# LSDOlab/femo_alpha

Measured on AMD Instinct MI355X. Metric: DOF/s (assembly+solve), forward solve of the RM shell; adjoint-gradient wallclock in adjoint_ms, higher is better.
Workload: dtype f64

## Files before the change

### femo_alpha_amd/_build.py

```python
from __future__ import annotations

import contextlib
import fcntl
import glob
import hashlib
import os
import shutil
import subprocess

CSRC = os.path.join(os.path.dirname(os.path.abspath(__file__)), "csrc")
INCLUDE = os.path.normpath(os.path.join(CSRC, "..", "..", "include"))
LIB = os.path.join(CSRC, "libfemo_hip.so")
HASHFILE = os.path.join(CSRC, "libfemo_hip.srchash")
SOURCES = ["femo_hip.hip"]
FLAGS = ["--offload-arch=gfx950", "-O3", "-std=c++17", "-fPIC", "-shared", "-munsafe-fp-atomics",
         "-Wno-unused-value"]


def dependencies():
    deps = sorted(glob.glob(os.path.join(CSRC, "*.hip")) + glob.glob(os.path.join(CSRC, "*.h"))
                  + [os.path.join(INCLUDE, "femo_hip.h")])
    return deps


# ... 51 lines not shown
            if os.path.exists(tmp):
                os.remove(tmp)
            raise RuntimeError("hipcc failed building libfemo_hip.so:\n" + res.stderr[-4000:])
        os.replace(tmp, LIB)
        _write_atomic(HASHFILE, digest + "\n")
    return LIB


SYM_LIB = os.path.join(CSRC, "libfemo_symbolic.so")
SYM_HASHFILE = os.path.join(CSRC, "libfemo_symbolic.srchash")
SYM_FLAGS = ["-O3", "-std=c++17", "-fPIC", "-shared", "-fopenmp"]


def symbolic_digest() -> str:
    h = hashlib.sha256(" ".join(SYM_FLAGS).encode())
    for d in (os.path.join(CSRC, "symbolic.cpp"), os.path.join(INCLUDE, "femo_symbolic.h")):
        h.update(os.path.basename(d).encode())
        with open(d, "rb") as fh:
            h.update(fh.read())
    return h.hexdigest()


def symbolic_needs_build() -> bool:
    if not os.path.exists(SYM_LIB) or not os.path.exists(SYM_HASHFILE):
        return True
    with open(SYM_HASHFILE) as fh:
        return fh.read().strip() != symbolic_digest()


def build_symbolic(force: bool = False) -> str:
    if not force and not symbolic_needs_build():
# ... 23 lines not shown
```

### femo_alpha_amd/csrc/femo_hip.hip

```cpp
#include "../../include/femo_hip.h"
#include "shell_device.h"
#include "frontal.h"
#include "sweeps_multi.h"
#include "shape_sens.h"
#include "residual_jvp.h"
#include "stress.h"
#include "stress_grad.h"
#include "stress_history.h"
#include "disp_history.h"
#include "ply_failure.h"
#include "ply_shear.h"
#include "field_jvp.h"
#include "ply_field_rev.h"
#include "layup.h"
#include "layup_mass.h"
#include "disp_aggregate.h"
#include "csr_map.h"
#include "hip_handles.h"

#include <hip/hip_runtime.h>

#include <algorithm>
#include <cmath>
#include <cstdio>
#include <cstdlib>
#include <cstring>
#include <string>
#include <utility>
#include <vector>

using namespace femo;

constexpr int WIDE_NP_DEFAULT = 512;
// ... 146 lines not shown
    DevBuf<double> scal;
    PinnedBuf<double> scal_host;
    bool jacobi_dirty = true;
    struct Options {
        int trailing = 0;
        int left_min = 64, left_max = 2048;
        int lookahead = 1, lookahead_cnt = 16;
        int super_panel = 512, super_panel_cnt = 64;
        int rows_fine_wg = 96;
        int narrow_fine_wg = 128;
        int fuse_rows = 1, fuse_rows_cnt = 2048;
        int fuse_rows_np = 2 * NBO;
        int sweep_graph = 0;
        int diag_v1_cnt = 512;
        int fused_schur = 1;
        int equilibrate = 0;
        int precond_nquad = 0;
        int grid_chunk = 32768;
        int wide_np = WIDE_NP_DEFAULT, wide_cnt = WIDE_CNT_DEFAULT;
        int strict = 1;
        int allow_pivot_repair = 0;
        int profile_verbose = 0;
        int diag_v1 = 0;
        int swork_slots = 8192;
        int xinv_small_cnt = 32;
        int bnd_tiled_nb = 1 << 30;
        int sweep_butterfly = 3;
        int sweep_w = 0;
        int assemble_fc = 1;
        int sweep_ahead = 2;
// ... 12 lines not shown
    double timing[5] = {0, 0, 0, 0, 0};
    std::string err;
    struct Frontal {
        bool ready = false, factored = false;
        bool have_factor = false;
        DevBuf<double> snap[6];
        bool snap_valid = false;
        bool w_mode = false;
        double* ahead_vec = nullptr;
        int ahead_levels = 0;
        bool x_inflight = false;
        int ntree = 0, nlevels = 0;
        std::vector<int> h_nf, h_npiv, h_level_off, h_level_nodes, h_level_maxnp, h_level_maxnb;
        std::vector<char> h_level_wide;
        DevBuf<int> nf, npiv, dofs, upmap, parent, left, right, level_nodes, elem_front, elem_map, info, cinv0, cinv1;
        DevBuf<long long> poff, soff, doff, linvoff, xoff;
        DevBuf<double> P, S, Linv, X, Xtmp, Swork;
        DevBuf<int> fel_off, fel;
        bool fc_ok = false;
        GraphExec sweep_graph;
        long long sweep_graph_key = -1;
        std::vector<long long> h_soff;
        long long p_doubles = 0, s_doubles = 0, linv_doubles = 0, x_doubles = 0;
        int swork_slots = 1;
        int max_nf = 0;
        int multi_nr = 4;
        double t_factor_ms = 0, t_assemble_ms = 0;
        int pivots_fixed = 0;
        bool profile = false;
        double prof_ms[8] = {0, 0, 0, 0, 0, 0, 0, 0};
// ... 449 lines not shown
    HIPCHK(c, hipStreamSynchronize(c->stream));
    float t_setup = 0, t_loop = 0;
    hipEventElapsedTime(&t_setup, c->ev[0], c->ev[1]);
    hipEventElapsedTime(&t_loop, c->ev[1], c->ev[2]);
    c->timing[0] = t_setup; c->timing[1] = t_loop; c->timing[2] = t_setup + t_loop; c->timing[3] = 0; c->timing[4] = napply;
    return finish_solve(c, "Jacobi-PCG", k, rr, bb, c->rtol * c->rtol * bb, iters, relres);
}


static FrontDev front_dev(const femo_ctx* c) {
    FrontDev fd;
    fd.ntree = c->fr.ntree; fd.nf = c->fr.nf; fd.npiv = c->fr.npiv; fd.poff = c->fr.poff; fd.soff = c->fr.soff; fd.doff = c->fr.doff;
    fd.dofs = c->fr.dofs; fd.upmap = c->fr.upmap; fd.parent = c->fr.parent; fd.child[0] = c->fr.left; fd.child[1] = c->fr.right;
    fd.linvoff = c->fr.linvoff; fd.xoff = c->fr.xoff; fd.P = c->fr.P; fd.S = c->fr.S; fd.Linv = c->fr.Linv; fd.X = c->fr.X; fd.Xtmp = c->fr.Xtmp;
    fd.cinv[0] = c->fr.cinv0; fd.cinv[1] = c->fr.cinv1;
    return fd;
}

struct ProfScope {
    femo_ctx* c; int cls; hipStream_t s; Event a, b;
    ProfScope(femo_ctx* c_, int cls_, hipStream_t s_ = nullptr) : c(c_), cls(cls_), s(s_ ? s_ : c_->stream.get()) {
        if (!c->fr.profile) return;
        hipEventCreate(a.out()); hipEventCreate(b.out());
        hipEventRecord(a, s);
    }
    ~ProfScope() {
        if (!c->fr.profile) return;
        hipEventRecord(b, s);
        c->fr.prof.push_back({std::move(a), std::move(b), cls, c->fr.cur_level, cls == 2 ? c->fr.last_fl : 0.0, cls == 2 ? c->fr.last_by : 0.0});
        c->fr.last_fl = c->fr.last_by = 0;
// ... 2017 lines not shown
    if (k == "trailing") { if (v < 0 || v > 2) return fail(c, "trailing: 0 auto, 1 left-looking, 2 right-looking"); o.trailing = v; }
    else if (k == "left_min") o.left_min = v;
    else if (k == "left_max") o.left_max = v;
    else if (k == "lookahead") o.lookahead = v != 0;
    else if (k == "lookahead_cnt") o.lookahead_cnt = v;
    else if (k == "super_panel") { if (v < 0) return fail(c, "super_panel: a column count (rounded down to whole 128-column panels; < 256 switches it off)"); o.super_panel = v; }
    else if (k == "super_panel_cnt") o.super_panel_cnt = v;
    else if (k == "rows_fine_wg") o.rows_fine_wg = v;
    else if (k == "narrow_fine_wg") o.narrow_fine_wg = v;
    else if (k == "diag_v1_cnt") o.diag_v1_cnt = v;
    else if (k == "sweep_graph") o.sweep_graph = v != 0;
    else if (k == "fuse_rows") o.fuse_rows = v != 0;
    else if (k == "fuse_rows_cnt") o.fuse_rows_cnt = v;
    else if (k == "fuse_rows_np") o.fuse_rows_np = v;
    else if (k == "fused_schur") o.fused_schur = v != 0;
    else if (k == "precond_nquad") { if (v != 0 && (v < 2 || v > 6)) return fail(c, "precond_nquad: 0 (the operator's rule) or 2..6"); o.precond_nquad = v; operator_changed(c); }
    else if (k == "equilibrate") { if (v < 0 || v > 2) return fail(c, "equilibrate: 0 off, 1 diag^-1/2, 2 nearest powers of two"); o.equilibrate = v; operator_changed(c); }
    else if (k == "grid_chunk") { if (v < 1 || v > 65535) return fail(c, "grid_chunk must be in 1..65535"); o.grid_chunk = v; }
    else if (k == "wide_np" || k == "wide_cnt") {
        if (c->fr.ready) return fail(c, "wide_np / wide_cnt shape the plan: set them before femo_set_frontal_plan");
        if (v < 0) return fail(c, "negative threshold");
        (k == "wide_np" ? o.wide_np : o.wide_cnt) = v;
    }
    else if (k == "strict") o.strict = v != 0;
    else if (k == "allow_pivot_repair") o.allow_pivot_repair = v != 0;
    else if (k == "stress_regularization") { if (value < 0) return fail(c, "stress_regularization: a coefficient >= 0 (the reference's is 0.5e3)"); c->stress_reg = value; }
    else if (k == "profile_verbose") o.profile_verbose = v != 0;
    else if (k == "diag_v1") { if (v < 0 || v > 3) return fail(c, "diag_v1: 0 auto, 1 round-2 kernel, 2 overlapped kernel, 3 the rule before the LDS diet"); o.diag_v1 = v; }
    else if (k == "profile") c->fr.profile = v != 0;
    else if (k == "bnd_tiled_nb") o.bnd_tiled_nb = v;
// ... 1133 lines not shown
    }
    {
        std::vector<int> inv0((size_t)ndofs_total, -1), inv1((size_t)ndofs_total, -1);
        for (int t = 0; t < ntree; ++t) {
            const int p = parent[t];
            if (p < 0) continue;
            std::vector<int>& inv = left[p] == t ? inv0 : inv1;
            if (left[p] != t && right[p] != t) return fail(c, "inconsistent frontal plan (parent / child links)");
            for (int k = npiv[t]; k < nf[t]; ++k) {
                const int pr = up_map[dof_off[t] + k];
                if (pr < 0 || pr >= nf[p]) return fail(c, "inconsistent frontal plan (up_map out of range)");
                inv[(size_t)dof_off[p] + pr] = k;
            }
        }
        UPI(fr.cinv0, inv0.data(), ndofs_total); UPI(fr.cinv1, inv1.data(), ndofs_total);
    }
    {
        std::vector<int> slot_of(ntree, 0);
        for (int i = 0; i < ntree; ++i) slot_of[level_nodes[i]] = i;
        const int cnt0 = level_off[1] - level_off[0];
        std::vector<int> fel_off(cnt0 + 1, 0), fel((size_t)std::max<long long>(c->nel, 1));
        fr.fc_ok = true;
        for (long long e = 0; e < c->nel && fr.fc_ok; ++e) {
            const int sl = slot_of[elem_front[e]] - level_off[0];
            if (sl < 0 || sl >= cnt0) fr.fc_ok = false; else ++fel_off[sl + 1];
        }
        if (fr.fc_ok) {
            for (int i = 0; i < cnt0; ++i) fel_off[i + 1] += fel_off[i];
            std::vector<int> fill(fel_off.begin(), fel_off.end() - 1);
            for (long long e = 0; e < c->nel; ++e) fel[fill[slot_of[elem_front[e]] - level_off[0]]++] = (int)e;
// ... 1822 lines not shown
```

### femo_alpha_amd/csrc/frontal.h

```cpp
#pragma once
#include "shell_device.h"

namespace femo {

constexpr int NB = 32;
constexpr int TS = 64;
constexpr int NBO = 128;
constexpr int SPD = 128;

struct FrontDev {
    int ntree;
    const int* nf;
    const int* npiv;
    const long long* poff;
    const long long* soff;
    const long long* doff;
    const int* dofs;
    const int* upmap;
    const int* parent;
    const int* child[2];
    const int* cinv[2];
    const long long* linvoff;
    const long long* xoff;
    double* P;
    double* S;
    double* Linv;
    double* X;
    double* Xtmp;
};

__device__ __host__ inline int ldp_of(int nf) { return (nf + 1) & ~1; }

struct FrontView {
    double* P;
    double* S;
    int nf, np;
// ... 297 lines not shown
    const long long dp = fd.doff[p];
    for (int i = threadIdx.x; i < 4 * TS; i += blockDim.x) {
        const int side = (i / TS) & 1, isc = i / (2 * TS), k = i % TS;
        const int g = (isc ? c0 : r0) + k;
        const int v = (g < nfp && (side ? ch1 : ch0) >= 0) ? fd.cinv[side][dp + g] : -1;
        if (isc) cmap[side][k] = v; else rmap[side][k] = v;
    }
    __syncthreads();
    const FrontView fp = front_view(fd, p);
    const FrontView f0 = front_view(fd, ch0 >= 0 ? ch0 : p), f1 = front_view(fd, ch1 >= 0 ? ch1 : p);
    const int* gd = fd.dofs + dp;
    const int lr = threadIdx.x % TS, lc0 = threadIdx.x / TS;
    const int r = r0 + lr;
    const int ra0 = rmap[0][lr], ra1 = rmap[1][lr];
    double v[TS / 4];
#pragma unroll
    for (int k = 0; k < TS / 4; ++k) {
        const int lc = lc0 + 4 * k, cc = c0 + lc;
        double x = 0.0;
        if (r < nfp && cc <= r && cc < c_end) {
            const int b0 = cmap[0][lc], b1 = cmap[1][lc];
            if (ra0 >= 0 && b0 >= 0) x += f0.col(min(ra0, b0))[max(ra0, b0)];
            if (ra1 >= 0 && b1 >= 0) x += f1.col(min(ra1, b1))[max(ra1, b1)];
        }
        v[k] = x;
    }
#pragma unroll
    for (int k = 0; k < TS / 4; ++k) {
        const int cc = c0 + lc0 + 4 * k;
        if (r < nfp && cc <= r && cc < c_end) {
            double x = v[k];
            if (mask && r == cc && r < npp && mask[gd[r]]) x = 1.0;
            fp.col(cc)[r] = x;
        }
    }
}

__device__ __forceinline__ double rl(double v, int lane) {
    int lo = __double2loint(v), hi = __double2hiint(v);
    lo = __builtin_amdgcn_readlane(lo, lane);
// ... 737 lines not shown

constexpr int LSTR = TS + 16;

struct TrailRange { int kc0, kw, col_lo, col_hi; };
__device__ __host__ inline TrailRange trail_range(int schur, int C0, int K0, int KW, int np, int nf) {
    TrailRange r{0, 0, 0, 0};
    if (schur != 1 && C0 >= np) return r;
    r.kc0 = schur >= 2 ? C0 : (schur ? 0 : K0);
    r.kw = schur >= 2 ? (KW < np - C0 ? KW : np - C0) : (schur ? np : C0 - K0);
    const int split = ((C0 + r.kw) & ~1) + NBO;
    r.col_lo = schur >= 2 ? (schur == 4 ? split : C0 + r.kw) : (schur ? np : C0);
    r.col_hi = schur == 0 ? (C0 + NBO < np ? C0 + NBO : np) : schur == 3 ? (split < nf ? split : nf) : nf;
    return r;
}

template <bool GATHER>
__global__ void __launch_bounds__(256, 4)
k_trailing_mfma(FrontDev fd, const int* __restrict__ level_nodes, int first, int C0, int schur, int K0, int KW,
                const unsigned char* __restrict__ mask) {
    int bxv = blockIdx.x, zv = blockIdx.z;
    {
        const int G = gridDim.x, n = gridDim.z;
        if (n >= 256 && (n & 7) == 0) {
            const int flat = bxv + G * zv, x = flat & 7, q = flat >> 3;
            zv = (q / G) * 8 + x; bxv = q % G;
        }
    }
    const int t = level_nodes[first + zv];
    const int np = fd.npiv[t];
    const int nf = fd.nf[t];
// ... 84 lines not shown
        cur ^= 1;
    }
    if (idle_quarter) return;
    bool cok[2][4];
#pragma unroll
    for (int a = 0; a < 2; ++a)
#pragma unroll
        for (int reg = 0; reg < 4; ++reg) {
            const int cc = cj + wc + 16 * a + l4 + 4 * reg;
            cok[a][reg] = cc >= col_lo && cc < col_hi;
        }
    auto col_ptr = [&](int a, int reg) {
        const int cc = cj + wc + 16 * a + l4 + 4 * reg;
        return cok[a][reg] ? fv.col(cc) : fv.P - (nf - 1);
    };
    double cv[2][2][4];
    if (!GATHER) {
        double* cp[2][4];
#pragma unroll
        for (int a = 0; a < 2; ++a)
#pragma unroll
            for (int reg = 0; reg < 4; ++reg) cp[a][reg] = col_ptr(a, reg);
#pragma unroll
        for (int a = 0; a < 2; ++a)
#pragma unroll
            for (int b = 0; b < 2; ++b)
#pragma unroll
                for (int reg = 0; reg < 4; ++reg) {
                    const int cc = cj + wc + 16 * a + l4 + 4 * reg;
                    const int r = ri + wr + 16 * b + l15;
                    const bool ok = cok[a][reg] && r < nf && r >= cc;
                    cv[a][b][reg] = cp[a][reg][ok ? r : nf - 1];
                }
    } else {
        const long long dp = fd.doff[t];
        int rr[2][2], cr[2][2][4];
        const double* Sc[2];
        int npc[2], nbc[2];
#pragma unroll
        for (int sd = 0; sd < 2; ++sd) {
            const int ch = fd.child[sd][t];
            const int chs = ch >= 0 ? ch : t;
            npc[sd] = fd.npiv[chs]; nbc[sd] = fd.nf[chs] - npc[sd];
            Sc[sd] = fd.S + fd.soff[chs];
#pragma unroll
            for (int b = 0; b < 2; ++b) {
                const int r = ri + wr + 16 * b + l15;
                rr[sd][b] = fd.cinv[sd][dp + min(r, nf - 1)];
                if (ch < 0 || r >= nf) rr[sd][b] = -1;
            }
#pragma unroll
            for (int a = 0; a < 2; ++a)
#pragma unroll
                for (int reg = 0; reg < 4; ++reg) {
                    const int cc = cj + wc + 16 * a + l4 + 4 * reg;
                    cr[sd][a][reg] = fd.cinv[sd][dp + min(cc, nf - 1)];
                    if (ch < 0 || !cok[a][reg]) cr[sd][a][reg] = -1;
                }
        }
        double g0[2][2][4], g1[2][2][4];
#pragma unroll
        for (int a = 0; a < 2; ++a)
#pragma unroll
            for (int b = 0; b < 2; ++b)
#pragma unroll
                for (int reg = 0; reg < 4; ++reg) {
                    const int cc = cj + wc + 16 * a + l4 + 4 * reg;
                    const int r = ri + wr + 16 * b + l15;
                    const bool tri = r >= cc;
                    {
                        const int x = rr[0][b], y = cr[0][a][reg];
                        const bool ok = tri && x >= 0 && y >= 0;
                        const int lo = min(x, y) - npc[0], hi = max(x, y) - npc[0];
                        g0[a][b][reg] = Sc[0][ok ? hi + (size_t)nbc[0] * lo : 0];
                        if (!ok) g0[a][b][reg] = 0.0;
                    }
                    {
                        const int x = rr[1][b], y = cr[1][a][reg];
                        const bool ok = tri && x >= 0 && y >= 0;
                        const int lo = min(x, y) - npc[1], hi = max(x, y) - npc[1];
                        g1[a][b][reg] = Sc[1][ok ? hi + (size_t)nbc[1] * lo : 0];
                        if (!ok) g1[a][b][reg] = 0.0;
                    }
                }
#pragma unroll
        for (int a = 0; a < 2; ++a)
#pragma unroll
            for (int b = 0; b < 2; ++b)
#pragma unroll
                for (int reg = 0; reg < 4; ++reg) cv[a][b][reg] = g0[a][b][reg] + g1[a][b][reg];
        if (mask && bx == 0) {
            const int* gd = fd.dofs + dp;
#pragma unroll
            for (int a = 0; a < 2; ++a)
#pragma unroll
                for (int b = 0; b < 2; ++b)
#pragma unroll
                    for (int reg = 0; reg < 4; ++reg) {
                        const int cc = cj + wc + 16 * a + l4 + 4 * reg;
                        const int r = ri + wr + 16 * b + l15;
                        if (r == cc && cok[a][reg] && cc < np && mask[gd[r]]) cv[a][b][reg] = 1.0;
                    }
        }
    }
#pragma unroll
    for (int a = 0; a < 2; ++a)
#pragma unroll
        for (int b = 0; b < 2; ++b)
#pragma unroll
            for (int reg = 0; reg < 4; ++reg) {
                const int cc = cj + wc + 16 * a + l4 + 4 * reg;
                const int r = ri + wr + 16 * b + l15;
                if (cok[a][reg] && r < nf && r >= cc) col_ptr(a, reg)[r] = cv[a][b][reg] - acc[a][b][reg];
            }
}

template <bool GATHER>
__global__ void __launch_bounds__(256, 2)
k_trailing_fine(FrontDev fd, const int* __restrict__ level_nodes, int first, int C0, int K0, const unsigned char* __restrict__ mask) {
    const int t = level_nodes[first + blockIdx.z];
    const int np = fd.npiv[t];
    const int nf = fd.nf[t];
    const TrailRange tr = trail_range(0, C0, K0, NBO, np, nf);
    const int kc0 = tr.kc0, kw = tr.kw, col_lo = tr.col_lo, col_hi = tr.col_hi;
    if (kw <= 0) return;
    constexpr int FT = 32;
    const int bxv = (int)blockIdx.x;
    const int by = bxv & 3, bx = bxv >> 2;
    const int cj = (col_lo & ~1) + by * FT;
// ... 34 lines not shown
    const int r = ri + wr + l15;
    bool cok[4];
    double* cp[4];
#pragma unroll
    for (int reg = 0; reg < 4; ++reg) {
        const int cc = cj + wc + l4 + 4 * reg;
        cok[reg] = cc >= col_lo && cc < col_hi && r < nf && r >= cc;
        cp[reg] = cok[reg] ? fv.col(cc) + r : fv.P;
    }
    double cv[4];
    if (!GATHER) {
#pragma unroll
        for (int reg = 0; reg < 4; ++reg) cv[reg] = *cp[reg];
    } else {
        const long long dp = fd.doff[t];
        double g[2][4];
#pragma unroll
        for (int sd = 0; sd < 2; ++sd) {
            const int ch = fd.child[sd][t];
            const int chs = ch >= 0 ? ch : t;
            const int npc = fd.npiv[chs], nbc = fd.nf[chs] - npc;
            const double* Sc = fd.S + fd.soff[chs];
            const int x = (ch >= 0 && r < nf) ? fd.cinv[sd][dp + r] : -1;
#pragma unroll
            for (int reg = 0; reg < 4; ++reg) {
                const int cc = cj + wc + l4 + 4 * reg;
                const int y = (ch >= 0 && cok[reg]) ? fd.cinv[sd][dp + cc] : -1;
                const bool ok = cok[reg] && x >= 0 && y >= 0;
                const int lo = min(x, y) - npc, hi = max(x, y) - npc;
                g[sd][reg] = Sc[ok ? hi + (size_t)nbc * lo : 0];
                if (!ok) g[sd][reg] = 0.0;
            }
        }
        const int* gd = fd.dofs + dp;
#pragma unroll
        for (int reg = 0; reg < 4; ++reg) {
            const int cc = cj + wc + l4 + 4 * reg;
            cv[reg] = g[0][reg] + g[1][reg];
            if (mask && r == cc && cok[reg] && cc < np && mask[gd[r]]) cv[reg] = 1.0;
        }
    }
#pragma unroll
    for (int reg = 0; reg < 4; ++reg)
        if (cok[reg]) *cp[reg] = cv[reg] - acc[reg];
}



constexpr int SMALL_PART = 512;

__global__ void __launch_bounds__(256, 4)
k_front_fwd_small(FrontDev fd, const int* __restrict__ level_nodes, double* __restrict__ v, double* __restrict__ yv) {
    const int t = level_nodes[blockIdx.x];
// ... 546 lines not shown
```

### femo_alpha_amd/csrc/symbolic.cpp

```cpp
#include <omp.h>

#include <algorithm>
#include <cmath>
#include <cstdint>
#include <cstdlib>
#include <cstring>
#include <map>
#include <numeric>
#include <string>
#include <vector>

#include "../../include/femo_symbolic.h"

namespace {

struct Plan {
    std::map<std::string, std::vector<int32_t>> i32;
    std::map<std::string, std::vector<int64_t>> i64;
    std::string error;
};

thread_local std::string g_error;

template <class T>
std::vector<T>& put(std::map<std::string, std::vector<T>>& m, const char* name) { return m[name]; }

}
// ... 411 lines not shown
    p->i32["lo"] = std::move(lo); p->i32["hi"] = std::move(hi); p->i32["left"] = std::move(left); p->i32["right"] = std::move(right);
    p->i32["parent"] = std::move(parent); p->i32["depth"] = std::move(depth); p->i32["height"] = std::move(height);
    p->i32["eorder"] = std::move(eorder); p->i32["epos"] = std::move(epos); p->i32["owner"] = std::move(owner);
    p->i32["piv_nodes"] = std::move(piv_nodes); p->i64["piv_off"] = std::move(piv_off);
    p->i32["bnd_nodes"] = std::move(bnd_nodes); p->i64["bnd_off"] = std::move(bnd_off);
    p->i32["npiv"] = std::move(npiv); p->i32["nf"] = std::move(nf); p->i64["dof_off"] = std::move(dof_off);
    p->i32["front_dofs"] = std::move(front_dofs); p->i32["up_map"] = std::move(up_map);
    p->i32["elem_front"] = std::move(elem_front); p->i32["elem_map"] = std::move(elem_map);
    p->i32["level_nodes"] = std::move(level_nodes); p->i64["level_off"] = std::move(level_off);
    p->i64["tail_delay_dofs"] = std::move(td_dofs); p->i32["tail_delay_saved"] = std::move(td_saved);
    p->i64["tail_delay_flops3"] = std::move(td_flops3);
    *out = p;
    return 0;
}

int femo_plan_build(femo_plan** out, int32_t nel, int32_t nP2, int32_t nV, int32_t npc, int32_t ndpc, const int32_t* cell_p2,
                    const double* cent, const int32_t* cell_dofs, int32_t leaf_size, int32_t min_depth) {
    return femo_plan_build_ex(out, nel, nP2, nV, npc, ndpc, cell_p2, cent, nullptr, cell_dofs, leaf_size, min_depth, 0, 0.0);
}

int64_t femo_plan_size(const femo_plan* p, const char* name) {
    if (!p || !name) return -1;
    auto a = p->i32.find(name);
    if (a != p->i32.end()) return (int64_t)a->second.size();
    auto b = p->i64.find(name);
    if (b != p->i64.end()) return (int64_t)b->second.size();
    return -1;
}

int femo_plan_itemsize(const femo_plan* p, const char* name) {
// ... 26 lines not shown
```

### femo_alpha_amd/solver/_native.py

```python
from __future__ import annotations

import ctypes as C

import numpy as np

from .. import _build

_lib = None
_i32p = C.POINTER(C.c_int32)

SIGNATURES = {
    "femo_plan_build": (C.c_int, [C.POINTER(C.c_void_p), C.c_int32, C.c_int32, C.c_int32, C.c_int32, C.c_int32, _i32p,
                                  C.POINTER(C.c_double), _i32p, C.c_int32, C.c_int32]),
    "femo_plan_build_ex": (C.c_int, [C.POINTER(C.c_void_p), C.c_int32, C.c_int32, C.c_int32, C.c_int32, C.c_int32, _i32p,
                                     C.POINTER(C.c_double), C.POINTER(C.c_double), _i32p, C.c_int32, C.c_int32, C.c_int32, C.c_double]),
    "femo_plan_build_ex2": (C.c_int, [C.POINTER(C.c_void_p), C.c_int32, C.c_int32, C.c_int32, C.c_int32, C.c_int32, _i32p,
                                      C.POINTER(C.c_double), C.POINTER(C.c_double), _i32p, C.c_int32, C.c_int32, C.c_int32, C.c_double, C.c_int32]),
    "femo_plan_size": (C.c_int64, [C.c_void_p, C.c_char_p]),
    "femo_plan_itemsize": (C.c_int, [C.c_void_p, C.c_char_p]),
    "femo_plan_get": (C.c_int, [C.c_void_p, C.c_char_p, C.c_void_p, C.c_int64]),
    "femo_plan_free": (None, [C.c_void_p]),
    "femo_plan_last_error": (C.c_char_p, []),
}

TAIL_DELAY_SIGNATURES = {
    "femo_tail_delay_plan_build": (C.c_int, SIGNATURES["femo_plan_build_ex2"][1] + [C.c_int32]),
}

ARRAYS = ("lo", "hi", "left", "right", "parent", "depth", "height", "eorder", "epos", "owner", "piv_nodes", "piv_off",
          "bnd_nodes", "bnd_off", "npiv", "nf", "dof_off", "front_dofs", "up_map", "elem_front", "elem_map", "level_nodes",
          "level_off", "tail_delay_dofs", "tail_delay_saved", "tail_delay_flops3")


def load():
    global _lib
    if _lib is None:
        path = _build.build_symbolic() if _build.symbolic_needs_build() else _build.SYM_LIB
        lib = C.CDLL(path)
        for name, (res, args) in {**SIGNATURES, **TAIL_DELAY_SIGNATURES}.items():
            fn = getattr(lib, name)
            fn.restype, fn.argtypes = res, args
        _lib = lib
    return _lib


def plan_arrays(mesh, leaf_size, min_depth=0, axis_rule=0, gap=0.0, node_order=0, tail_max=0):
    lib = load()
    cr = getattr(mesh, "element", "") == "CG2CR1"
    nV_lib = mesh.nE if cr else mesh.nV
    cell_p2 = np.ascontiguousarray(mesh.cell_p2, dtype=np.int32)
    cell_dofs = np.ascontiguousarray(mesh.cell_dofs(), dtype=np.int32)
    if cr:
        nV, nE = mesh.nV, mesh.nE
        to_lib = np.concatenate([nE + np.arange(nV), np.arange(nE)]).astype(np.int32)
# ... 23 lines not shown
            if lib.femo_plan_get(h, name.encode(), a.ctypes.data_as(C.c_void_p), a.nbytes):
                raise RuntimeError(lib.femo_plan_last_error().decode())
            out[name] = a
    finally:
        lib.femo_plan_free(h)
    out["elem_map"] = out["elem_map"].reshape(mesh.nel, -1)
    if cr:
        fd = out["front_dofs"].astype(np.int64)
        isu = fd < mesh.ndof_u
        fd[isu] = 3 * from_lib[fd[isu] // 3] + fd[isu] % 3
        out["front_dofs"] = fd.astype(out["front_dofs"].dtype)
        for k in ("piv_nodes", "bnd_nodes"):
            out[k] = from_lib[out[k]].astype(out[k].dtype)
        out["owner"] = out["owner"][to_lib]
    return out
```

### femo_alpha_amd/solver/symbolic.py

```python
from __future__ import annotations

import numpy as np

from ..mesh import ShellMesh

__all__ = ["FrontalPlan", "Tree", "analyse", "build_plan", "rank_plan"]


class FrontalPlan:

    def summary(self):
        nf, npv = self.nf, self.npiv
        flops = float(np.sum(npv.astype(np.float64) * nf.astype(np.float64) ** 2
                             - npv.astype(np.float64) ** 2 * nf + npv.astype(np.float64) ** 3 / 3.0))
        out = dict(fronts=int(self.ntree), levels=int(self.nlevels), leaves=int(self.nleaves),
                   max_front=int(nf.max()), max_pivots=int(npv.max()),
                   front_doubles=int(self.front_off[-1]), front_GB=float(self.front_off[-1] * 8 / 1e9),
                   factor_doubles=int(np.sum(nf.astype(np.int64) * npv)), factor_gflop=flops / 1e9)
        td = getattr(self, "tail_delay", None)
        if td is not None and int(np.sum(td["saved"])):
            f0, f1 = td["flops3"]
            out.update(delayed_dofs=int(np.sum(td["dofs"])), panels_saved={int(h): int(s) for h, s in enumerate(td["saved"]) if s},
                       delay_flop_change=float(f1 - f0) / float(f0))
        return out
# ... 358 lines not shown
    ends = np.cumsum(lens)
    ndofs_seg = csum[ends] - csum[ends - lens]
    dofs_all = _node_dofs(nodes_all, nV, ndof_u)
    seg_off = np.concatenate([[0], np.cumsum(ndofs_seg)])
    dof_lists = [dofs_all[seg_off[2 * t]:seg_off[2 * t + 2]] for t in range(T.ntree)]
    npiv = ndofs_seg[0::2]
    leaf_of_pos = np.zeros(mesh.nel, dtype=np.int64)
    for t in np.nonzero(T.left < 0)[0]:
        leaf_of_pos[T.lo[t]:T.hi[t]] = t
    plan = _assemble_plan(dof_lists, npiv, T.parent, T.left, T.right, T.height, leaf_of_pos[T.epos], mesh.cell_dofs())
    plan.eorder = T.eorder.astype(np.int32)
    plan.tail_delay = T.tail_delay
    return plan


def rank_plan(mesh, T: Tree, rank, nranks):
    return _rank_plan(mesh, T, rank, nranks)


def _rank_plan(mesh, T: Tree, rank, nranks):
    d = int(np.log2(nranks))
    if 2 ** d != nranks:
        raise ValueError("number of ranks must be a power of two")
    roots = np.nonzero(T.depth == d)[0]
    roots = roots[np.argsort(T.lo[roots], kind="stable")]
    if roots.size != nranks or np.any(T.depth[T.left < 0] < d):
        raise ValueError("tree is not deep enough for this many ranks")
    root = int(roots[rank])
    nVg, ndof_ug = mesh.nV, mesh.ndof_u
    cr = getattr(mesh, "element", "") == "CG2CR1"
# ... 76 lines not shown
```

### include/femo_symbolic.h

```cpp
#ifndef FEMO_SYMBOLIC_H
#define FEMO_SYMBOLIC_H
#include <stdint.h>
#ifdef __cplusplus
extern "C" {
#endif

typedef struct femo_plan femo_plan;

int femo_plan_build(femo_plan** out, int32_t nel, int32_t nP2, int32_t nV, int32_t npc, int32_t ndpc, const int32_t* cell_p2,
                    const double* cent, const int32_t* cell_dofs, int32_t leaf_size, int32_t min_depth);
int femo_plan_build_ex(femo_plan** out, int32_t nel, int32_t nP2, int32_t nV, int32_t npc, int32_t ndpc, const int32_t* cell_p2,
                       const double* cent, const double* cext, const int32_t* cell_dofs, int32_t leaf_size, int32_t min_depth,
                       int32_t axis_rule, double gap_coeff);
int femo_plan_build_ex2(femo_plan** out, int32_t nel, int32_t nP2, int32_t nV, int32_t npc, int32_t ndpc, const int32_t* cell_p2,
                        const double* cent, const double* cext, const int32_t* cell_dofs, int32_t leaf_size, int32_t min_depth,
                        int32_t axis_rule, double gap_coeff, int32_t node_order);
int femo_tail_delay_plan_build(femo_plan** out, int32_t nel, int32_t nP2, int32_t nV, int32_t npc, int32_t ndpc, const int32_t* cell_p2,
                               const double* cent, const double* cext, const int32_t* cell_dofs, int32_t leaf_size, int32_t min_depth,
                               int32_t axis_rule, double gap_coeff, int32_t node_order, int32_t tail_max);
int64_t femo_plan_size(const femo_plan* p, const char* name);
int femo_plan_itemsize(const femo_plan* p, const char* name);
int femo_plan_get(const femo_plan* p, const char* name, void* dst, int64_t nbytes);
void femo_plan_free(femo_plan* p);
const char* femo_plan_last_error(void);

#ifdef __cplusplus
}
#endif
#endif
```

Baseline: 63.88 million.

## Use monotone child-map fast path for extend-add gather in frontal factorization

Precomputes, per front, whether each child's boundary-to-parent map is strictly increasing, and uploads these flags to the device. When both children are monotone, the trailing-update and Schur gather kernels skip the min/max symmetric index swap. They use precomputed byte offsets, bitmasks and 32-bit address arithmetic, and mask values instead of branching on them. The epilogue store also switches to 32-bit offsets when the front fits. This adds host preprocessing and more register pressure, and it relies on monotonicity and size limits for correctness.

```diff
diff --git a/femo_alpha_amd/_build.py b/femo_alpha_amd/_build.py
--- a/femo_alpha_amd/_build.py
+++ b/femo_alpha_amd/_build.py
@@ -89,7 +89,7 @@
 
 def symbolic_digest() -> str:
     h = hashlib.sha256(" ".join(SYM_FLAGS).encode())
-    for d in (os.path.join(CSRC, "symbolic.cpp"), os.path.join(INCLUDE, "femo_symbolic.h")):
+    for d in (os.path.join(CSRC, "symbolic.cpp"), os.path.join(CSRC, "child_maps.h"), os.path.join(INCLUDE, "femo_symbolic.h")):
         h.update(os.path.basename(d).encode())
         with open(d, "rb") as fh:
             h.update(fh.read())
diff --git a/femo_alpha_amd/csrc/child_maps.h b/femo_alpha_amd/csrc/child_maps.h
--- /dev/null
+++ b/femo_alpha_amd/csrc/child_maps.h
@@ -0,0 +1,24 @@
+#pragma once
+#include <cstdint>
+
+namespace femo {
+
+inline bool up_map_increasing(const int32_t* up_bnd, int64_t nb) {
+    for (int64_t k = 1; k < nb; ++k)
+        if (up_bnd[k] <= up_bnd[k - 1]) return false;
+    return true;
+}
+
+inline void child_maps_increasing(int32_t ntree, const int32_t* npiv, const int32_t* nf, const int64_t* dof_off, const int32_t* parent,
+                                  const int32_t* left, const int32_t* right, const int32_t* up_map, int32_t* flags) {
+    for (int32_t t = 0; t < ntree; ++t) flags[t] = 3;
+    for (int32_t t = 0; t < ntree; ++t) {
+        const int32_t p = parent[t];
+        if (p < 0 || p >= ntree) continue;
+        if (up_map_increasing(up_map + dof_off[t] + npiv[t], (int64_t)nf[t] - npiv[t])) continue;
+        if (left[p] == t) flags[p] &= ~1;
+        else if (right[p] == t) flags[p] &= ~2;
+    }
+}
+
+}
diff --git a/femo_alpha_amd/csrc/femo_hip.hip b/femo_alpha_amd/csrc/femo_hip.hip
--- a/femo_alpha_amd/csrc/femo_hip.hip
+++ b/femo_alpha_amd/csrc/femo_hip.hip
@@ -17,6 +17,7 @@
 #include "disp_aggregate.h"
 #include "csr_map.h"
 #include "hip_handles.h"
+#include "child_maps.h"
 
 #include <hip/hip_runtime.h>
 
@@ -193,6 +194,7 @@
         int sweep_graph = 0;
         int diag_v1_cnt = 512;
         int fused_schur = 1;
+        int gather_mono = 1;
         int equilibrate = 0;
         int precond_nquad = 0;
         int grid_chunk = 32768;
@@ -235,6 +237,7 @@
         std::vector<int> h_nf, h_npiv, h_level_off, h_level_nodes, h_level_maxnp, h_level_maxnb;
         std::vector<char> h_level_wide;
         DevBuf<int> nf, npiv, dofs, upmap, parent, left, right, level_nodes, elem_front, elem_map, info, cinv0, cinv1;
+        DevBuf<int> cmono;
         DevBuf<long long> poff, soff, doff, linvoff, xoff;
         DevBuf<double> P, S, Linv, X, Xtmp, Swork;
         DevBuf<int> fel_off, fel;
@@ -714,6 +717,7 @@
     fd.dofs = c->fr.dofs; fd.upmap = c->fr.upmap; fd.parent = c->fr.parent; fd.child[0] = c->fr.left; fd.child[1] = c->fr.right;
     fd.linvoff = c->fr.linvoff; fd.xoff = c->fr.xoff; fd.P = c->fr.P; fd.S = c->fr.S; fd.Linv = c->fr.Linv; fd.X = c->fr.X; fd.Xtmp = c->fr.Xtmp;
     fd.cinv[0] = c->fr.cinv0; fd.cinv[1] = c->fr.cinv1;
+    fd.cmono = c->fr.cmono + (c->opt.gather_mono ? 0 : c->fr.ntree);
     return fd;
 }
 
@@ -2761,6 +2765,7 @@
     else if (k == "fuse_rows_cnt") o.fuse_rows_cnt = v;
     else if (k == "fuse_rows_np") o.fuse_rows_np = v;
     else if (k == "fused_schur") o.fused_schur = v != 0;
+    else if (k == "gather_mono") o.gather_mono = v != 0;
     else if (k == "precond_nquad") { if (v != 0 && (v < 2 || v > 6)) return fail(c, "precond_nquad: 0 (the operator's rule) or 2..6"); o.precond_nquad = v; operator_changed(c); }
     else if (k == "equilibrate") { if (v < 0 || v > 2) return fail(c, "equilibrate: 0 off, 1 diag^-1/2, 2 nearest powers of two"); o.equilibrate = v; operator_changed(c); }
     else if (k == "grid_chunk") { if (v < 1 || v > 65535) return fail(c, "grid_chunk must be in 1..65535"); o.grid_chunk = v; }
@@ -3924,6 +3929,11 @@
             }
         }
         UPI(fr.cinv0, inv0.data(), ndofs_total); UPI(fr.cinv1, inv1.data(), ndofs_total);
+        std::vector<int32_t> mono(2 * (size_t)ntree, 0);
+        femo::child_maps_increasing(ntree, npiv, nf, dof_off, parent, left, right, up_map, mono.data());
+        for (int t = 0; t < ntree; ++t)
+            if (parent[t] >= 0 && nf[t] - npiv[t] > (1 << 14)) mono[parent[t]] = 0;
+        UPI(fr.cmono, mono.data(), 2 * (size_t)ntree);
     }
     {
         std::vector<int> slot_of(ntree, 0);
diff --git a/femo_alpha_amd/csrc/frontal.h b/femo_alpha_amd/csrc/frontal.h
--- a/femo_alpha_amd/csrc/frontal.h
+++ b/femo_alpha_amd/csrc/frontal.h
@@ -20,6 +20,7 @@
     const int* parent;
     const int* child[2];
     const int* cinv[2];
+    const int* cmono;
     const long long* linvoff;
     const long long* xoff;
     double* P;
@@ -347,6 +348,31 @@
     const int r = r0 + lr;
     const int ra0 = rmap[0][lr], ra1 = rmap[1][lr];
     double v[TS / 4];
+    if (fd.cmono[p] == 3) {
+        const bool diag = ti == tj;
+        double g[2][TS / 4];
+#pragma unroll
+        for (int sd = 0; sd < 2; ++sd) {
+            const FrontView& fc = sd ? f1 : f0;
+            const int npc = fc.np, nbc = fc.nf - fc.np;
+            const int ra = sd ? ra1 : ra0;
+            const unsigned rowb = 8u * (unsigned)(max(ra, npc) - npc);
+            bool cok[TS / 4];
+#pragma unroll
+            for (int k = 0; k < TS / 4; ++k) {
+                const int lc = lc0 + 4 * k;
+                const int b = __builtin_amdgcn_readfirstlane(cmap[sd][lc]);
+                cok[k] = b >= 0 && c0 + lc < c_end;
+                const char* cb = reinterpret_cast<const char*>(fc.S + (size_t)nbc * (size_t)(max(b, npc) - npc));
+                g[sd][k] = *reinterpret_cast<const double*>(cb + rowb);
+            }
+#pragma unroll
+            for (int k = 0; k < TS / 4; ++k)
+                if (!(ra >= 0 && cok[k] && (!diag || c0 + lc0 + 4 * k <= r))) g[sd][k] = 0.0;
+        }
+#pragma unroll
+        for (int k = 0; k < TS / 4; ++k) v[k] = (0.0 + g[0][k]) + g[1][k];
+    } else {
 #pragma unroll
     for (int k = 0; k < TS / 4; ++k) {
         const int lc = lc0 + 4 * k, cc = c0 + lc;
@@ -357,6 +383,7 @@
             if (ra1 >= 0 && b1 >= 0) x += f1.col(min(ra1, b1))[max(ra1, b1)];
         }
         v[k] = x;
+    }
     }
 #pragma unroll
     for (int k = 0; k < TS / 4; ++k) {
@@ -1124,6 +1151,138 @@
     return r;
 }
 
+
+template <int NA, int NR>
+struct GatherMono {
+    const char* Sc[2];
+    unsigned colb[2][NA][4], rowb[2][NR];
+    unsigned em[2][NR];
+};
+
+template <int NA, int NR, bool DIAG>
+__device__ __forceinline__ void gather_mono_prepare(const FrontDev& fd, int t, long long dp, int nf, int col_lo, int col_hi, const int (&r)[NR],
+                                                    const int (&cc)[NA][4], GatherMono<NA, NR>& gm) {
+    int outm[NA][4];
+#pragma unroll
+    for (int a = 0; a < NA; ++a)
+#pragma unroll
+        for (int reg = 0; reg < 4; ++reg) outm[a][reg] = ((cc[a][reg] - col_lo) | (col_hi - 1 - cc[a][reg])) >> 31;
+#pragma unroll
+    for (int sd = 0; sd < 2; ++sd) {
+        const int ch = fd.child[sd][t];
+        const int chs = ch >= 0 ? ch : t;
+        const int nochild = ch >> 31;
+        const int npc = fd.npiv[chs], nbc = fd.nf[chs] - npc;
+        gm.Sc[sd] = reinterpret_cast<const char*>(fd.S + fd.soff[chs]);
+        const char* inv = reinterpret_cast<const char*>(fd.cinv[sd] + dp);
+        unsigned colbits = 0u;
+#pragma unroll
+        for (int a = 0; a < NA; ++a)
+#pragma unroll
+            for (int reg = 0; reg < 4; ++reg) {
+                const int y = *reinterpret_cast<const int*>(inv + 4u * (unsigned)min(cc[a][reg], nf - 1)) | nochild | outm[a][reg];
+                colbits |= ((unsigned)~y >> 31) << (4 * a + reg);
+                gm.colb[sd][a][reg] = __umul24(8u * (unsigned)nbc, (unsigned)(max(y, npc) - npc));
+            }
+#pragma unroll
+        for (int b = 0; b < NR; ++b) {
+            const int x = *reinterpret_cast<const int*>(inv + 4u * (unsigned)min(r[b], nf - 1)) | nochild | ((nf - 1 - r[b]) >> 31);
+            gm.em[sd][b] = colbits & (unsigned)~(x >> 31);
+            gm.rowb[sd][b] = 8u * (unsigned)(max(x, npc) - npc);
+        }
+    }
+    if (DIAG) {
+#pragma unroll
+        for (int b = 0; b < NR; ++b) {
+            unsigned tri = 0u;
+#pragma unroll
+            for (int a = 0; a < NA; ++a)
+#pragma unroll
+                for (int reg = 0; reg < 4; ++reg) tri |= ((unsigned)(cc[a][reg] - 1 - r[b]) >> 31) << (4 * a + reg);
+            gm.em[0][b] &= tri; gm.em[1][b] &= tri;
+        }
+    }
+}
+
+template <int NA, int NR>
+__device__ __forceinline__ void gather_mono_fetch(const GatherMono<NA, NR>& gm, int a, double (&out)[NR][4]) {
+    double g[2][NR][4];
+#pragma unroll
+    for (int sd = 0; sd < 2; ++sd)
+#pragma unroll
+        for (int b = 0; b < NR; ++b)
+#pragma unroll
+            for (int reg = 0; reg < 4; ++reg) g[sd][b][reg] = *reinterpret_cast<const double*>(gm.Sc[sd] + (gm.colb[sd][a][reg] + gm.rowb[sd][b]));
+#pragma unroll
+    for (int b = 0; b < NR; ++b)
+#pragma unroll
+        for (int reg = 0; reg < 4; ++reg) {
+            double gs[2];
+#pragma unroll
+            for (int sd = 0; sd < 2; ++sd) {
+                const int m = (int)(gm.em[sd][b] << (31 - (4 * a + reg))) >> 31;
+                gs[sd] = __hiloint2double(__double2hiint(g[sd][b][reg]) & m, __double2loint(g[sd][b][reg]) & m);
+            }
+            out[b][reg] = gs[0] + gs[1];
+        }
+}
+
+template <int NA, int NR>
+__device__ __forceinline__ void gather_tile_any(const FrontDev& fd, int t, long long dp, int nf, const int (&r)[NR], const int (&cc)[NA][4],
+                                                const bool (&ccok)[NA][4], double (&cv)[NA][NR][4]) {
+    int rr[2][NR], cr[2][NA][4];
+    const double* Sc[2];
+    int npc[2], nbc[2];
+#pragma unroll
+    for (int sd = 0; sd < 2; ++sd) {
+        const int ch = fd.child[sd][t];
+        const int chs = ch >= 0 ? ch : t;
+        npc[sd] = fd.npiv[chs]; nbc[sd] = fd.nf[chs] - npc[sd];
+        Sc[sd] = fd.S + fd.soff[chs];
+#pragma unroll
+        for (int b = 0; b < NR; ++b) {
+            rr[sd][b] = fd.cinv[sd][dp + min(r[b], nf - 1)];
+            if (ch < 0 || r[b] >= nf) rr[sd][b] = -1;
+        }
+#pragma unroll
+        for (int a = 0; a < NA; ++a)
+#pragma unroll
+            for (int reg = 0; reg < 4; ++reg) {
+                cr[sd][a][reg] = fd.cinv[sd][dp + min(cc[a][reg], nf - 1)];
+                if (ch < 0 || !ccok[a][reg]) cr[sd][a][reg] = -1;
+            }
+    }
+    double g0[NA][NR][4], g1[NA][NR][4];
+#pragma unroll
+    for (int a = 0; a < NA; ++a)
+#pragma unroll
+        for (int b = 0; b < NR; ++b)
+#pragma unroll
+            for (int reg = 0; reg < 4; ++reg) {
+                const bool tri = r[b] >= cc[a][reg];
+                {
+                    const int x = rr[0][b], y = cr[0][a][reg];
+                    const bool ok = tri && x >= 0 && y >= 0;
+                    const int lo = min(x, y) - npc[0], hi = max(x, y) - npc[0];
+                    g0[a][b][reg] = Sc[0][ok ? hi + (size_t)nbc[0] * lo : 0];
+                    if (!ok) g0[a][b][reg] = 0.0;
+                }
+                {
+                    const int x = rr[1][b], y = cr[1][a][reg];
+                    const bool ok = tri && x >= 0 && y >= 0;
+                    const int lo = min(x, y) - npc[1], hi = max(x, y) - npc[1];
+                    g1[a][b][reg] = Sc[1][ok ? hi + (size_t)nbc[1] * lo : 0];
+                    if (!ok) g1[a][b][reg] = 0.0;
+                }
+            }
+#pragma unroll
+    for (int a = 0; a < NA; ++a)
+#pragma unroll
+        for (int b = 0; b < NR; ++b)
+#pragma unroll
+            for (int reg = 0; reg < 4; ++reg) cv[a][b][reg] = g0[a][b][reg] + g1[a][b][reg];
+}
+
 template <bool GATHER>
 __global__ void __launch_bounds__(256, 4)
 k_trailing_mfma(FrontDev fd, const int* __restrict__ level_nodes, int first, int C0, int schur, int K0, int KW,
@@ -1238,6 +1397,70 @@
         const int cc = cj + wc + 16 * a + l4 + 4 * reg;
         return cok[a][reg] ? fv.col(cc) : fv.P - (nf - 1);
     };
+    const int st_side = (col_lo >= np && nf - np <= (1 << 14)) ? 1 : (col_hi <= np && (size_t)ldp * (size_t)np < (size_t)(1u << 28)) ? 0 : -1;
+    const int st_ld = st_side == 1 ? nf - np : ldp, st_c0 = st_side == 1 ? np : 0;
+    char* const st_base = reinterpret_cast<char*>(st_side == 1 ? fv.S : fv.P);
+    auto finish = [&](int a, const double (&cva)[2][4]) {
+        double x[2][4];
+#pragma unroll
+        for (int b = 0; b < 2; ++b)
+#pragma unroll
+            for (int reg = 0; reg < 4; ++reg) x[b][reg] = cva[b][reg];
+        if (GATHER && mask && bx == 0) {
+            const int* gd = fd.dofs + fd.doff[t];
+#pragma unroll
+            for (int b = 0; b < 2; ++b)
+#pragma unroll
+                for (int reg = 0; reg < 4; ++reg) {
+                    const int cc = cj + wc + 16 * a + l4 + 4 * reg;
+                    const int r = ri + wr + 16 * b + l15;
+                    if (r == cc && cok[a][reg] && cc < np && mask[gd[r]]) x[b][reg] = 1.0;
+                }
+        }
+        if (st_side >= 0) {
+            unsigned co[4], ro[2];
+#pragma unroll
+            for (int reg = 0; reg < 4; ++reg) co[reg] = 8u * (unsigned)st_ld * (unsigned)(cj + wc + 16 * a + l4 + 4 * reg - st_c0);
+#pragma unroll
+            for (int b = 0; b < 2; ++b) ro[b] = 8u * (unsigned)(ri + wr + 16 * b + l15 - st_c0);
+#pragma unroll
+            for (int b = 0; b < 2; ++b)
+#pragma unroll
+                for (int reg = 0; reg < 4; ++reg) {
+                    const int cc = cj + wc + 16 * a + l4 + 4 * reg;
+                    const int r = ri + wr + 16 * b + l15;
+                    if (cok[a][reg] && r < nf && r >= cc) *reinterpret_cast<double*>(st_base + (co[reg] + ro[b])) = x[b][reg] - acc[a][b][reg];
+                }
+            return;
+        }
+#pragma unroll
+        for (int b = 0; b < 2; ++b)
+#pragma unroll
+            for (int reg = 0; reg < 4; ++reg) {
+                const int cc = cj + wc + 16 * a + l4 + 4 * reg;
+                const int r = ri + wr + 16 * b + l15;
+                if (cok[a][reg] && r < nf && r >= cc) col_ptr(a, reg)[r] = x[b][reg] - acc[a][b][reg];
+            }
+    };
+    int gr[2], gc[2][4];
+#pragma unroll
+    for (int b = 0; b < 2; ++b) gr[b] = ri + wr + 16 * b + l15;
+#pragma unroll
+    for (int a = 0; a < 2; ++a)
+#pragma unroll
+        for (int reg = 0; reg < 4; ++reg) gc[a][reg] = cj + wc + 16 * a + l4 + 4 * reg;
+    if (GATHER && fd.cmono[t] == 3) {
+        GatherMono<2, 2> gm;
+        if (bx == 0) gather_mono_prepare<2, 2, true>(fd, t, fd.doff[t], nf, col_lo, col_hi, gr, gc, gm);
+        else gather_mono_prepare<2, 2, false>(fd, t, fd.doff[t], nf, col_lo, col_hi, gr, gc, gm);
+#pragma unroll
+        for (int a = 0; a < 2; ++a) {
+            double cva[2][4];
+            gather_mono_fetch<2, 2>(gm, a, cva);
+            finish(a, cva);
+        }
+        return;
+    }
     double cv[2][2][4];
     if (!GATHER) {
         double* cp[2][4];
@@ -1256,87 +1479,9 @@
                     const bool ok = cok[a][reg] && r < nf && r >= cc;
                     cv[a][b][reg] = cp[a][reg][ok ? r : nf - 1];
                 }
-    } else {
-        const long long dp = fd.doff[t];
-        int rr[2][2], cr[2][2][4];
-        const double* Sc[2];
-        int npc[2], nbc[2];
-#pragma unroll
-        for (int sd = 0; sd < 2; ++sd) {
-            const int ch = fd.child[sd][t];
-            const int chs = ch >= 0 ? ch : t;
-            npc[sd] = fd.npiv[chs]; nbc[sd] = fd.nf[chs] - npc[sd];
-            Sc[sd] = fd.S + fd.soff[chs];
-#pragma unroll
-            for (int b = 0; b < 2; ++b) {
-                const int r = ri + wr + 16 * b + l15;
-                rr[sd][b] = fd.cinv[sd][dp + min(r, nf - 1)];
-                if (ch < 0 || r >= nf) rr[sd][b] = -1;
-            }
-#pragma unroll
-            for (int a = 0; a < 2; ++a)
-#pragma unroll
-                for (int reg = 0; reg < 4; ++reg) {
-                    const int cc = cj + wc + 16 * a + l4 + 4 * reg;
-                    cr[sd][a][reg] = fd.cinv[sd][dp + min(cc, nf - 1)];
-                    if (ch < 0 || !cok[a][reg]) cr[sd][a][reg] = -1;
-                }
-        }
-        double g0[2][2][4], g1[2][2][4];
-#pragma unroll
-        for (int a = 0; a < 2; ++a)
-#pragma unroll
-            for (int b = 0; b < 2; ++b)
-#pragma unroll
-                for (int reg = 0; reg < 4; ++reg) {
-                    const int cc = cj + wc + 16 * a + l4 + 4 * reg;
-                    const int r = ri + wr + 16 * b + l15;
-                    const bool tri = r >= cc;
-                    {
-                        const int x = rr[0][b], y = cr[0][a][reg];
-                        const bool ok = tri && x >= 0 && y >= 0;
-                        const int lo = min(x, y) - npc[0], hi = max(x, y) - npc[0];
-                        g0[a][b][reg] = Sc[0][ok ? hi + (size_t)nbc[0] * lo : 0];
-                        if (!ok) g0[a][b][reg] = 0.0;
-                    }
-                    {
-                        const int x = rr[1][b], y = cr[1][a][reg];
-                        const bool ok = tri && x >= 0 && y >= 0;
-                        const int lo = min(x, y) - npc[1], hi = max(x, y) - npc[1];
-                        g1[a][b][reg] = Sc[1][ok ? hi + (size_t)nbc[1] * lo : 0];
-                        if (!ok) g1[a][b][reg] = 0.0;
-                    }
-                }
-#pragma unroll
-        for (int a = 0; a < 2; ++a)
-#pragma unroll
-            for (int b = 0; b < 2; ++b)
-#pragma unroll
-                for (int reg = 0; reg < 4; ++reg) cv[a][b][reg] = g0[a][b][reg] + g1[a][b][reg];
-        if (mask && bx == 0) {
-            const int* gd = fd.dofs + dp;
-#pragma unroll
-            for (int a = 0; a < 2; ++a)
-#pragma unroll
-                for (int b = 0; b < 2; ++b)
-#pragma unroll
-                    for (int reg = 0; reg < 4; ++reg) {
-                        const int cc = cj + wc + 16 * a + l4 + 4 * reg;
-                        const int r = ri + wr + 16 * b + l15;
-                        if (r == cc && cok[a][reg] && cc < np && mask[gd[r]]) cv[a][b][reg] = 1.0;
-                    }
-        }
-    }
-#pragma unroll
-    for (int a = 0; a < 2; ++a)
-#pragma unroll
-        for (int b = 0; b < 2; ++b)
-#pragma unroll
-            for (int reg = 0; reg < 4; ++reg) {
-                const int cc = cj + wc + 16 * a + l4 + 4 * reg;
-                const int r = ri + wr + 16 * b + l15;
-                if (cok[a][reg] && r < nf && r >= cc) col_ptr(a, reg)[r] = cv[a][b][reg] - acc[a][b][reg];
-            }
+    } else gather_tile_any<2, 2>(fd, t, fd.doff[t], nf, gr, gc, cok, cv);
+#pragma unroll
+    for (int a = 0; a < 2; ++a) finish(a, cv[a]);
 }
 
 template <bool GATHER>
@@ -1401,29 +1546,25 @@
         for (int reg = 0; reg < 4; ++reg) cv[reg] = *cp[reg];
     } else {
         const long long dp = fd.doff[t];
-        double g[2][4];
-#pragma unroll
-        for (int sd = 0; sd < 2; ++sd) {
-            const int ch = fd.child[sd][t];
-            const int chs = ch >= 0 ? ch : t;
-            const int npc = fd.npiv[chs], nbc = fd.nf[chs] - npc;
-            const double* Sc = fd.S + fd.soff[chs];
-            const int x = (ch >= 0 && r < nf) ? fd.cinv[sd][dp + r] : -1;
-#pragma unroll
-            for (int reg = 0; reg < 4; ++reg) {
-                const int cc = cj + wc + l4 + 4 * reg;
-                const int y = (ch >= 0 && cok[reg]) ? fd.cinv[sd][dp + cc] : -1;
-                const bool ok = cok[reg] && x >= 0 && y >= 0;
-                const int lo = min(x, y) - npc, hi = max(x, y) - npc;
-                g[sd][reg] = Sc[ok ? hi + (size_t)nbc * lo : 0];
-                if (!ok) g[sd][reg] = 0.0;
-            }
-        }
+        int gr[1] = {r}, gc[1][4];
+        bool ccok[1][4];
+        double g[1][1][4];
+#pragma unroll
+        for (int reg = 0; reg < 4; ++reg) {
+            gc[0][reg] = cj + wc + l4 + 4 * reg;
+            ccok[0][reg] = gc[0][reg] >= col_lo && gc[0][reg] < col_hi;
+        }
+        if (fd.cmono[t] == 3) {
+            GatherMono<1, 1> gm;
+            if (bx == 0) gather_mono_prepare<1, 1, true>(fd, t, dp, nf, col_lo, col_hi, gr, gc, gm);
+            else gather_mono_prepare<1, 1, false>(fd, t, dp, nf, col_lo, col_hi, gr, gc, gm);
+            gather_mono_fetch<1, 1>(gm, 0, g[0]);
+        } else gather_tile_any<1, 1>(fd, t, dp, nf, gr, gc, ccok, g);
         const int* gd = fd.dofs + dp;
 #pragma unroll
         for (int reg = 0; reg < 4; ++reg) {
             const int cc = cj + wc + l4 + 4 * reg;
-            cv[reg] = g[0][reg] + g[1][reg];
+            cv[reg] = g[0][0][reg];
             if (mask && r == cc && cok[reg] && cc < np && mask[gd[r]]) cv[reg] = 1.0;
         }
     }
diff --git a/femo_alpha_amd/csrc/symbolic.cpp b/femo_alpha_amd/csrc/symbolic.cpp
--- a/femo_alpha_amd/csrc/symbolic.cpp
+++ b/femo_alpha_amd/csrc/symbolic.cpp
@@ -11,6 +11,7 @@
 #include <vector>
 
 #include "../../include/femo_symbolic.h"
+#include "child_maps.h"
 
 namespace {
 
@@ -452,6 +453,16 @@
     return 0;
 }
 
+int femo_child_maps_increasing(int32_t ntree, const int32_t* npiv, const int32_t* nf, const int64_t* dof_off, const int32_t* parent,
+                               const int32_t* left, const int32_t* right, const int32_t* up_map, int32_t* flags) {
+    if (ntree < 1 || !npiv || !nf || !dof_off || !parent || !left || !right || !up_map || !flags) {
+        g_error = "femo_child_maps_increasing: bad arguments";
+        return 1;
+    }
+    femo::child_maps_increasing(ntree, npiv, nf, dof_off, parent, left, right, up_map, flags);
+    return 0;
+}
+
 int femo_plan_build(femo_plan** out, int32_t nel, int32_t nP2, int32_t nV, int32_t npc, int32_t ndpc, const int32_t* cell_p2,
                     const double* cent, const int32_t* cell_dofs, int32_t leaf_size, int32_t min_depth) {
     return femo_plan_build_ex(out, nel, nP2, nV, npc, ndpc, cell_p2, cent, nullptr, cell_dofs, leaf_size, min_depth, 0, 0.0);
diff --git a/femo_alpha_amd/solver/_native.py b/femo_alpha_amd/solver/_native.py
--- a/femo_alpha_amd/solver/_native.py
+++ b/femo_alpha_amd/solver/_native.py
@@ -27,6 +27,11 @@
     "femo_tail_delay_plan_build": (C.c_int, SIGNATURES["femo_plan_build_ex2"][1] + [C.c_int32]),
 }
 
+_i64p = C.POINTER(C.c_int64)
+CHILD_MAPS_SIGNATURES = {
+    "femo_child_maps_increasing": (C.c_int, [C.c_int32, _i32p, _i32p, _i64p, _i32p, _i32p, _i32p, _i32p, _i32p]),
+}
+
 ARRAYS = ("lo", "hi", "left", "right", "parent", "depth", "height", "eorder", "epos", "owner", "piv_nodes", "piv_off",
           "bnd_nodes", "bnd_off", "npiv", "nf", "dof_off", "front_dofs", "up_map", "elem_front", "elem_map", "level_nodes",
           "level_off", "tail_delay_dofs", "tail_delay_saved", "tail_delay_flops3")
@@ -37,7 +42,7 @@
     if _lib is None:
         path = _build.build_symbolic() if _build.symbolic_needs_build() else _build.SYM_LIB
         lib = C.CDLL(path)
-        for name, (res, args) in {**SIGNATURES, **TAIL_DELAY_SIGNATURES}.items():
+        for name, (res, args) in {**SIGNATURES, **TAIL_DELAY_SIGNATURES, **CHILD_MAPS_SIGNATURES}.items():
             fn = getattr(lib, name)
             fn.restype, fn.argtypes = res, args
         _lib = lib
@@ -91,3 +96,15 @@
             out[k] = from_lib[out[k]].astype(out[k].dtype)
         out["owner"] = out["owner"][to_lib]
     return out
+
+
+def child_maps_increasing(plan):
+    lib = load()
+    i32 = lambda a: np.ascontiguousarray(a, dtype=np.int32)
+    npiv, nf, parent, left, right, up = (i32(getattr(plan, k)) for k in ("npiv", "nf", "parent", "left", "right", "up_map"))
+    dof_off = np.ascontiguousarray(plan.dof_off, dtype=np.int64)
+    flags = np.empty(int(plan.ntree), dtype=np.int32)
+    p = lambda a: a.ctypes.data_as(_i32p)
+    if lib.femo_child_maps_increasing(int(plan.ntree), p(npiv), p(nf), dof_off.ctypes.data_as(_i64p), p(parent), p(left), p(right), p(up), p(flags)):
+        raise RuntimeError(lib.femo_plan_last_error().decode())
+    return flags
diff --git a/femo_alpha_amd/solver/symbolic.py b/femo_alpha_amd/solver/symbolic.py
--- a/femo_alpha_amd/solver/symbolic.py
+++ b/femo_alpha_amd/solver/symbolic.py
@@ -396,6 +396,25 @@
     return plan
 
 
+def child_maps_increasing(plan, impl="native"):
+    if impl == "native":
+        from . import _native
+        return _native.child_maps_increasing(plan)
+    flags = np.full(int(plan.ntree), 3, dtype=np.int32)
+    for t in range(int(plan.ntree)):
+        p = int(plan.parent[t])
+        if p < 0:
+            continue
+        rows = np.asarray(plan.up_map[plan.dof_off[t] + plan.npiv[t]:plan.dof_off[t + 1]], dtype=np.int64)
+        if np.all(np.diff(rows) > 0):
+            continue
+        if plan.left[p] == t:
+            flags[p] &= ~1
+        elif plan.right[p] == t:
+            flags[p] &= ~2
+    return flags
+
+
 def rank_plan(mesh, T: Tree, rank, nranks):
     return _rank_plan(mesh, T, rank, nranks)
 
diff --git a/include/femo_symbolic.h b/include/femo_symbolic.h
--- a/include/femo_symbolic.h
+++ b/include/femo_symbolic.h
@@ -18,6 +18,8 @@
 int femo_tail_delay_plan_build(femo_plan** out, int32_t nel, int32_t nP2, int32_t nV, int32_t npc, int32_t ndpc, const int32_t* cell_p2,
                                const double* cent, const double* cext, const int32_t* cell_dofs, int32_t leaf_size, int32_t min_depth,
                                int32_t axis_rule, double gap_coeff, int32_t node_order, int32_t tail_max);
+int femo_child_maps_increasing(int32_t ntree, const int32_t* npiv, const int32_t* nf, const int64_t* dof_off, const int32_t* parent,
+                               const int32_t* left, const int32_t* right, const int32_t* up_map, int32_t* flags);
 int64_t femo_plan_size(const femo_plan* p, const char* name);
 int femo_plan_itemsize(const femo_plan* p, const char* name);
 int femo_plan_get(const femo_plan* p, const char* name, void* dst, int64_t nbytes);
```

Measured after the change: 64.85 million, median of 6. 1.5% higher.
